# BaguaSys/bagua-core

Hardware: AMD Instinct MI355X
Metric: GiB/s fp32 gradient encode+decode (device-resident); 1/2/4/8-GPU compressed all-reduce GiB/s (higher is better)
Workload: dtype f32 -> u8

## Files before the change

bagua-core_amd/csrc/kernels/minmax_resident.hip:

```cpp
#include <hip/hip_runtime.h>
#include <stdio.h>
#include <stdlib.h>

#include <chrono>
#include <map>
#include <mutex>
#include <set>
#include <thread>
#include <utility>

#include "codec_common.hpp"
#include "launch_util.hpp"

namespace bagua {

constexpr int kResMaxGrid = 1024;
constexpr int kResSlots = 64;
constexpr int kResLanes = 8;

struct ResidentSlot {
    uint64_t ticket[kResLanes][16];
    uint64_t drained[kResLanes][16];
    uint64_t gave_up;
    uint64_t pad0[15];
    uint64_t gran[2 * kResMaxGrid];
};
static_assert(sizeof(ResidentSlot) % 64 == 0, "slot alignment");

struct ResidentArgs {
    const void* in;
    int64_t cs;
    int target;
    int nact;
    int bpc;
    int grid;
    uint8_t* out;
    int64_t chunk_offset;
    int64_t out_bytes;
    int num_chunks;
    ResidentSlot* slot;
    uint64_t timeout_ticks;
    uint64_t* trace;
};

__device__ __forceinline__ void trace_stamp(const ResidentArgs& a, int g, int k) {
    if (a.trace != nullptr && threadIdx.x == 0) a.trace[8 * g + k] = wall_clock64();
}

__device__ __forceinline__ uint32_t tag_of_ticket(uint64_t ticket, int grid, int lane) {
    const uint64_t per_launch = (uint64_t)((grid - lane + kResLanes - 1) / kResLanes);
    return (uint32_t)((ticket / per_launch) % 0xffffffffull) + 1u;
}

template <typename T, int BLOCK>
struct SliceGeom {
    using S = typename T::storage;
    int c;
    int cl;
    int b;
    const S* src;
    uint8_t* seg;
    uint8_t* payload;
    int64_t j0;
    int64_t nvec;
    int64_t v0, v1;
    bool last;

    __device__ __forceinline__ SliceGeom(const ResidentArgs& a, int g) {
        constexpr int N = Vec<T>::N;
        cl = g / a.bpc;
        b = g - cl * a.bpc;
        c = a.target < 0 ? cl : a.target;
        src = static_cast<const S*>(a.in) + (int64_t)c * a.cs;
        seg = a.out + (int64_t)c * a.chunk_offset;
        payload = seg + 32;
        const int al = common_alignment<T>((uintptr_t)src, (uintptr_t)payload);
        j0 = al < a.cs ? al : a.cs;
        nvec = (a.cs - j0) / N;
        const int64_t per = ((nvec + a.bpc - 1) / a.bpc + BLOCK - 1) / BLOCK * BLOCK;
        v0 = (int64_t)b * per;
        v0 = v0 < nvec ? v0 : nvec;
        v1 = v0 + per < nvec ? v0 + per : nvec;
        last = (b == a.bpc - 1);
    }
};

template <typename T>
__device__ __forceinline__ void fold_vec(const uint4& r, uint32_t& lo, uint32_t& hi) {
    float f[Vec<T>::N];
    unpack16<T>(r, f);
#pragma unroll
    for (int i = 0; i < Vec<T>::N; ++i) {
        const int32_t k = f2key(f[i]);
        lo = min(lo, min_space_key(k));
        hi = min(hi, max_space_key(k));
    }
}

template <typename T, int BLOCK>
__device__ __forceinline__ void fold_scalars(const ResidentArgs& a, const SliceGeom<T, BLOCK>& s, uint32_t& lo,
                                             uint32_t& hi) {
    constexpr int N = Vec<T>::N;
    const int t = (int)threadIdx.x;
    for (int64_t j = t; j < s.j0; j += BLOCK) {
        const int32_t k = f2key(T::to_f(s.src[j]));
        lo = min(lo, min_space_key(k));
        hi = min(hi, max_space_key(k));
    }
    for (int64_t j = s.j0 + s.nvec * N + t; j < a.cs; j += BLOCK) {
        const int32_t k = f2key(T::to_f(s.src[j]));
        lo = min(lo, min_space_key(k));
        hi = min(hi, max_space_key(k));
    }
}

template <int SB, int BLOCK, bool NT = false>
__device__ __forceinline__ void load_tile(const uint4* __restrict__ v, int64_t base, int t, uint4 (&r)[SB]) {
#pragma unroll
    for (int j = 0; j < SB; ++j) r[j] = NT ? nt_load16(&v[base + j * BLOCK + t]) : v[base + j * BLOCK + t];
}

template <typename T>
__device__ __forceinline__ void quant_store(const uint4& r, const QParams& q, uint8_t* dst) {
    float f[Vec<T>::N];
    unpack16<T>(r, f);
    quant_store_vec<T>(f, q, dst);
}

template <typename T, int BLOCK>
__device__ void write_extras(const ResidentArgs& a, const SliceGeom<T, BLOCK>& s, float mn, float mx,
                             const QParams& q) {
    using S = typename T::storage;
    constexpr int N = Vec<T>::N;
    const int t = (int)threadIdx.x;
    if (s.b == 0 && t < 32) {
        const uint32_t bmn = sizeof(S) == 4 ? __float_as_uint(mn) : (uint32_t)T::from_f(mn);
        const uint32_t bmx = sizeof(S) == 4 ? __float_as_uint(mx) : (uint32_t)T::from_f(mx);
        uint32_t hb = 0;
        if (t < (int)sizeof(S)) hb = (bmn >> (8 * t)) & 0xff;
        else if (t < 2 * (int)sizeof(S)) hb = (bmx >> (8 * (t - (int)sizeof(S)))) & 0xff;
        s.seg[t] = (uint8_t)hb;
    }
    if (!s.last) return;
    for (int64_t j = 32 + a.cs + t; j < a.chunk_offset; j += BLOCK) s.seg[j] = 0;
    if (a.target < 0 && s.c == a.num_chunks - 1)
        for (int64_t j = (int64_t)a.num_chunks * a.chunk_offset + t; j < a.out_bytes; j += BLOCK) a.out[j] = 0;
    for (int64_t j = t; j < s.j0; j += BLOCK) s.payload[j] = (uint8_t)quant(T::to_f(s.src[j]), q);
    for (int64_t j = s.j0 + s.nvec * N + t; j < a.cs; j += BLOCK)
        s.payload[j] = (uint8_t)quant(T::to_f(s.src[j]), q);
}

__device__ __forceinline__ bool sweep_chunk(const ResidentArgs& a, int cl, uint32_t tag, uint64_t deadline,
                                            uint32_t& lo, uint32_t& hi, bool bounded) {
    const int lane = lane_id();
    const uint64_t* g = a.slot->gran + 2 * (int64_t)cl * a.bpc;
    const int n = 2 * a.bpc;
    for (;;) {
        bool ok = true;
        uint32_t l = 0xffffffffu, h = 0xffffffffu;
        for (int i = lane; i < n; i += kWave) {
            const uint64_t x = __hip_atomic_load(g + i, __ATOMIC_RELAXED, __HIP_MEMORY_SCOPE_AGENT);
            ok &= (uint32_t)(x >> 32) == tag;
            if (i & 1) h = min(h, (uint32_t)x);
            else l = min(l, (uint32_t)x);
        }
        if (__all(ok)) {
            lo = wave_umin(l);
            hi = wave_umin(h);
            return true;
        }
        if (bounded && (uint64_t)wall_clock64() > deadline) return false;
        __builtin_amdgcn_s_sleep(2);
    }
}

template <typename T, int BLOCK, bool LEAN = false>
__device__ void fold_missing_slices(const ResidentArgs& a, int cl, uint32_t tag, uint32_t& lo, uint32_t& hi) {
    const int t = (int)threadIdx.x;
    for (int b = 0; b < a.bpc; ++b) {
        const int gg = cl * a.bpc + b;
        const uint64_t* gr = a.slot->gran + 2 * (int64_t)gg;
        const uint64_t x0 = __hip_atomic_load(gr, __ATOMIC_RELAXED, __HIP_MEMORY_SCOPE_AGENT);
        const uint64_t x1 = __hip_atomic_load(gr + 1, __ATOMIC_RELAXED, __HIP_MEMORY_SCOPE_AGENT);
        if ((uint32_t)(x0 >> 32) == tag && (uint32_t)(x1 >> 32) == tag) {
            lo = min(lo, (uint32_t)x0);
            hi = min(hi, (uint32_t)x1);
            continue;
        }
        const SliceGeom<T, BLOCK> sg(a, gg);
        const uint4* __restrict__ v = reinterpret_cast<const uint4*>(sg.src + sg.j0);
        if constexpr (LEAN) {
#pragma unroll 1
            for (int64_t i = sg.v0 + t; i < sg.v1; i += BLOCK) fold_vec<T>(v[i], lo, hi);
        } else {
            for (int64_t i = sg.v0 + t; i < sg.v1; i += BLOCK) fold_vec<T>(v[i], lo, hi);
        }
        if (sg.last) fold_scalars<T, BLOCK>(a, sg, lo, hi);
    }
}


template <int BLOCK>
__device__ __forceinline__ uint32_t draw_tag(const ResidentArgs& a, int lane_c, int t, uint32_t* scratch) {
    constexpr int W = BLOCK / kWave;
    if (t == 0) {
        const uint64_t ticket = __hip_atomic_fetch_add(&a.slot->ticket[lane_c][0], (uint64_t)1, __ATOMIC_RELAXED,
                                                       __HIP_MEMORY_SCOPE_AGENT);
        scratch[2 * W] = tag_of_ticket(ticket, a.grid, lane_c);
    }
    __syncthreads();
    return scratch[2 * W];
}

__device__ __forceinline__ void let_go_of_slot(const ResidentArgs& a, int lane_c, int t) {
    if (t == 0)
        __hip_atomic_fetch_add(&a.slot->drained[lane_c][0], (uint64_t)1, __ATOMIC_RELAXED,
                               __HIP_MEMORY_SCOPE_AGENT);
}

__device__ __forceinline__ void finish(const ResidentArgs& a, int g, int lane_c, int t) {
    if (a.trace != nullptr) {
        __syncthreads();
        trace_stamp(a, g, 3);
    }
    let_go_of_slot(a, lane_c, t);
}

template <int K, int ROW0, int BLOCK, bool NT, int M>
__device__ __forceinline__ void load_rows(const uint4* v, int64_t base, int64_t vl, int t,
                                          uint4 (&r)[M]) {
    static_assert(K <= M, "more rows than registers");
#pragma unroll
    for (int k = 0; k < K; ++k) {
        const int64_t i = base + (int64_t)(ROW0 + k) * BLOCK + t;
        r[k] = NT ? nt_load16(&v[i < vl ? i : vl]) : v[i < vl ? i : vl];
    }
}

template <typename T, int K, bool FENCE4, int M>
__device__ __forceinline__ void fold_rows(const uint4 (&r)[M], uint32_t& lo, uint32_t& hi) {
#pragma unroll
    for (int k = 0; k < K; ++k) {
        fold_vec<T>(r[k], lo, hi);
        if (FENCE4 && k % 4 == 3) __builtin_amdgcn_sched_barrier(0);
    }
}

template <typename T, int BLOCK, int H, int SB, int ROW0, bool NT>
__device__ __forceinline__ void fold_and_park(const uint4* v, int64_t v0, int64_t vl, int t,
                                              uint4 (&cur)[SB], uint4* park, uint32_t& lo, uint32_t& hi) {
    uint4 nxt[SB];
#pragma unroll
    for (int kb = 0; kb < H; kb += SB) {
#pragma unroll
        for (int j = 0; j < SB; ++j) {
            if (kb + SB + j < H) {
                const int64_t i = v0 + (int64_t)(ROW0 + kb + SB + j) * BLOCK + t;
                nxt[j] = NT ? nt_load16(&v[i < vl ? i : vl]) : v[i < vl ? i : vl];
            }
        }
#pragma unroll
        for (int j = 0; j < SB; ++j) {
            if (kb + j < H) {
                fold_vec<T>(cur[j], lo, hi);
                park[(kb + j) * BLOCK + t] = cur[j];
            }
        }
#pragma unroll
        for (int j = 0; j < SB; ++j) cur[j] = nxt[j];
    }
}

template <typename T, int BLOCK, int SB>
__device__ __forceinline__ void fold_stream_ascending(const uint4* v, int64_t stream0, int64_t nfull, int64_t last, int t,
                                                      uint4 (&ra)[SB], uint4 (&rb)[SB], uint32_t& lo,
                                                      uint32_t& hi) {
    constexpr int64_t tile = (int64_t)SB * BLOCK;
    for (int64_t i = 0; i < nfull; i += 2) {
        load_tile<SB, BLOCK>(v, stream0 + (i + 1 < nfull ? i + 1 : last) * tile, t, rb);
        fold_rows<T, SB, false>(ra, lo, hi);
        load_tile<SB, BLOCK>(v, stream0 + (i + 2 < nfull ? i + 2 : last) * tile, t, ra);
        if (i + 1 < nfull) fold_rows<T, SB, false>(rb, lo, hi);
    }
}

template <int BLOCK>
__device__ __forceinline__ void workgroup_umin(uint32_t& lo, uint32_t& hi, int t, int w, uint32_t* scratch) {
    constexpr int W = BLOCK / kWave;
    lo = wave_umin(lo);
    hi = wave_umin(hi);
    if (lane_id() == 0) { scratch[w] = lo; scratch[W + w] = hi; }
    __syncthreads();
    if (t == 0) {
#pragma unroll
        for (int i = 1; i < W; ++i) { lo = min(lo, scratch[i]); hi = min(hi, scratch[W + i]); }
    }
}

template <int BLOCK>
__device__ __forceinline__ void publish_partials(const ResidentArgs& a, int g, uint32_t tag, uint32_t lo, uint32_t hi,
                                                 int t, int w, uint32_t* scratch) {
    workgroup_umin<BLOCK>(lo, hi, t, w, scratch);
    if (t == 0) {
        uint64_t* mine = a.slot->gran + 2 * (int64_t)g;
        __hip_atomic_store(mine, ((uint64_t)tag << 32) | lo, __ATOMIC_RELAXED, __HIP_MEMORY_SCOPE_AGENT);
        __hip_atomic_store(mine + 1, ((uint64_t)tag << 32) | hi, __ATOMIC_RELAXED, __HIP_MEMORY_SCOPE_AGENT);
    }
}

struct MinMax {
    float mn, mx;
};

template <typename T, int BLOCK, bool LEAN>
__device__ __forceinline__ MinMax exchange_minmax(const ResidentArgs& a, int cl, uint32_t tag, int t, int w,
                                                  uint32_t* scratch) {
    constexpr int W = BLOCK / kWave;
    if (w == 0) {
        const uint64_t deadline = wall_clock64() + a.timeout_ticks;
        uint32_t l = 0, h = 0;
        const bool ok = sweep_chunk(a, cl, tag, deadline, l, h, true);
        if (lane_id() == 0) {
            scratch[2 * W + 1] = ok ? 1u : 0u;
            scratch[2 * W + 2] = l;
            scratch[2 * W + 3] = h;
        }
    }
    __syncthreads();
    if (scratch[2 * W + 1] == 0u) {
        if (t == 0) __hip_atomic_fetch_add(&a.slot->gave_up, (uint64_t)1, __ATOMIC_RELAXED, __HIP_MEMORY_SCOPE_AGENT);
        uint32_t l = 0xffffffffu, h = 0xffffffffu;
        fold_missing_slices<T, BLOCK, LEAN>(a, cl, tag, l, h);
        workgroup_umin<BLOCK>(l, h, t, w, scratch);
        if (t == 0) {
            scratch[2 * W + 2] = l;
            scratch[2 * W + 3] = h;
        }
        __syncthreads();
    }
    return MinMax{from_min_space(scratch[2 * W + 2]), from_max_space(scratch[2 * W + 3])};
}

template <int ON_CHIP>
__device__ __forceinline__ int on_chip_count(int64_t v0, int64_t v1) {
    return (int)(v1 - v0 < (int64_t)ON_CHIP ? (v1 > v0 ? v1 - v0 : 0) : (int64_t)ON_CHIP);
}

template <typename T, int BLOCK, int K, int ROW0, bool FENCE4, int M>
__device__ __forceinline__ void quant_rows(const uint4 (&r)[M], const QParams& q, uint8_t* vd) {
    constexpr int N = Vec<T>::N;
#pragma unroll
    for (int k = 0; k < K; ++k) {
        quant_store<T>(r[k], q, vd + (int64_t)(ROW0 + k) * BLOCK * N);
        if (FENCE4 && k % 4 == 3) __builtin_amdgcn_sched_barrier(0);
    }
}

template <typename T, int BLOCK, int K, int ROW0, int M>
__device__ __forceinline__ void quant_rows_guarded(const uint4 (&r)[M], int nloc, int t, const QParams& q,
                                                   uint8_t* vd) {
    constexpr int N = Vec<T>::N;
#pragma unroll
    for (int k = 0; k < K; ++k)
        if ((ROW0 + k) * BLOCK + t < nloc) quant_store<T>(r[k], q, vd + (int64_t)(ROW0 + k) * BLOCK * N);
}

template <typename T, int BLOCK, int H, int SB, int ROW0>
__device__ __forceinline__ void quant_parked(const uint4* park, int t, const QParams& q, uint8_t* vd) {
    constexpr int N = Vec<T>::N;
#pragma unroll
    for (int kb = 0; kb < H; kb += SB) {
        uint4 r[SB];
#pragma unroll
        for (int j = 0; j < SB; ++j)
            if (kb + j < H) r[j] = park[(kb + j) * BLOCK + t];
#pragma unroll
        for (int j = 0; j < SB; ++j)
            if (kb + j < H) quant_store<T>(r[j], q, vd + (int64_t)(ROW0 + kb + j) * BLOCK * N);
    }
}

template <typename T, int BLOCK, int H, int ROW0>
__device__ __forceinline__ void quant_parked_guarded(const uint4* park, int nloc, int t, const QParams& q,
                                                     uint8_t* vd) {
    constexpr int N = Vec<T>::N;
#pragma unroll
    for (int k = 0; k < H; ++k)
        if ((ROW0 + k) * BLOCK + t < nloc)
            quant_store<T>(park[k * BLOCK + t], q, vd + (int64_t)(ROW0 + k) * BLOCK * N);
}

template <typename T, int BLOCK, int SB>
__device__ __forceinline__ void quant_top_tile(const uint4 (&r)[SB], int64_t top, int64_t v1, int t,
                                               const QParams& q, uint8_t* vdst) {
    constexpr int N = Vec<T>::N;
#pragma unroll
    for (int j = 0; j < SB; ++j) {
        const int64_t i = top + j * BLOCK + t;
        if (i < v1) quant_store<T>(r[j], q, vdst + i * N);
    }
}

template <typename T, int BLOCK, int SB, bool NT>
__device__ __forceinline__ void quant_stream_descending(const uint4* v, int64_t stream0, int64_t nfull, int t,
                                                        const QParams& q, uint8_t* vdst, uint4 (&qa)[SB],
                                                        uint4 (&qb)[SB]) {
    constexpr int N = Vec<T>::N;
    constexpr int64_t tile = (int64_t)SB * BLOCK;
    for (int64_t i = nfull - 1; i >= 0; i -= 2) {
        load_tile<SB, BLOCK, NT>(v, stream0 + (i >= 1 ? i - 1 : 0) * tile, t, qb);
        const int64_t ba = stream0 + i * tile;
#pragma unroll
        for (int j = 0; j < SB; ++j) quant_store<T>(qa[j], q, vdst + (ba + j * BLOCK + t) * N);
        load_tile<SB, BLOCK, NT>(v, stream0 + (i >= 2 ? i - 2 : 0) * tile, t, qa);
        if (i >= 1) {
            const int64_t bb = ba - tile;
#pragma unroll
            for (int j = 0; j < SB; ++j) quant_store<T>(qb[j], q, vdst + (bb + j * BLOCK + t) * N);
        }
    }
}

template <typename T, int BLOCK, int SB, bool NT>
__device__ __forceinline__ void quant_stream_ascending(const uint4* v, int64_t stream0, int64_t nfull, int t,
                                                       const QParams& q, uint8_t* vdst, uint4 (&qa)[SB],
                                                       uint4 (&qb)[SB]) {
    constexpr int N = Vec<T>::N;
    constexpr int64_t tile = (int64_t)SB * BLOCK;
    for (int64_t i = 0; i < nfull; i += 2) {
        load_tile<SB, BLOCK, NT>(v, stream0 + (i + 1 < nfull ? i + 1 : nfull - 1) * tile, t, qb);
        const int64_t ba = stream0 + i * tile;
#pragma unroll
        for (int j = 0; j < SB; ++j) quant_store<T>(qa[j], q, vdst + (ba + j * BLOCK + t) * N);
        load_tile<SB, BLOCK, NT>(v, stream0 + (i + 2 < nfull ? i + 2 : nfull - 1) * tile, t, qa);
        if (i + 1 < nfull) {
            const int64_t bb = ba + tile;
#pragma unroll
            for (int j = 0; j < SB; ++j) quant_store<T>(qb[j], q, vdst + (bb + j * BLOCK + t) * N);
        }
    }
}

template <typename T, int BLOCK, int R, int H, int SB, int NTM>
__global__ __launch_bounds__(BLOCK, 1) void minmax_resident_encode_kernel(ResidentArgs a) {
    constexpr int N = Vec<T>::N;
    constexpr bool NT = (NTM & 1) != 0;
    constexpr bool NT1 = (NTM & 2) != 0;
    extern __shared__ __attribute__((aligned(16))) uint4 smem[];
    uint4* park = smem;
    uint32_t* scratch = reinterpret_cast<uint32_t*>(smem + H * BLOCK);
    const int t = (int)threadIdx.x;
    const int g = (int)blockIdx.x;
    const int lane_c = g % kResLanes;

    const uint32_t tag = draw_tag<BLOCK>(a, lane_c, t, scratch);
    trace_stamp(a, g, 0);
    if (g >= a.nact * a.bpc) {
        let_go_of_slot(a, lane_c, t);
        return;
    }

    const SliceGeom<T, BLOCK> s(a, g);
    const uint4* __restrict__ v = reinterpret_cast<const uint4*>(s.src + s.j0);
    const int64_t v0 = s.v0, v1 = s.v1;
    const int64_t stream0 = v0 + (int64_t)(R + H) * BLOCK;

    uint32_t lo = min_space(T::init_max());
    uint32_t hi = max_space(-T::init_max());
    uint4 held[R > 0 ? R : 1];
    if (v1 > v0) {
        const int64_t vl = v1 - 1;
        load_rows<R, 0, BLOCK, NT1>(v, v0, vl, t, held);
        uint4 cur[SB];
        load_rows<(H < SB ? H : SB), R, BLOCK, NT1>(v, v0, vl, t, cur);
        fold_rows<T, R, false>(held, lo, hi);
        fold_and_park<T, BLOCK, H, SB, R, NT1>(v, v0, vl, t, cur, park, lo, hi);
        const int64_t tile = (int64_t)SB * BLOCK;
        const int64_t nfull = v1 > stream0 ? (v1 - stream0) / tile : 0;
        if (nfull > 0) {
            uint4 ra[SB], rb[SB];
            load_tile<SB, BLOCK>(v, stream0, t, ra);
            fold_stream_ascending<T, BLOCK, SB>(v, stream0, nfull, nfull - 1, t, ra, rb, lo, hi);
        }
        for (int j = 0; j < SB; ++j) {
            const int64_t i = stream0 + nfull * tile + j * BLOCK + t;
            if (i < v1) fold_vec<T>(v[i], lo, hi);
        }
    }
    if (s.last) fold_scalars<T, BLOCK>(a, s, lo, hi);
    const int w = t / kWave;
    publish_partials<BLOCK>(a, g, tag, lo, hi, t, w, scratch);

    const int64_t tile2 = (int64_t)SB * BLOCK;
    const int64_t nfull2 = v1 > stream0 ? (v1 - stream0) / tile2 : 0;
    uint4 pre[SB], pre2[SB];
    if (nfull2 > 0) load_tile<SB, BLOCK, NT>(v, stream0 + (nfull2 - 1) * tile2, t, pre);
    if (nfull2 > 1) load_tile<SB, BLOCK, NT>(v, stream0 + (nfull2 - 2) * tile2, t, pre2);

    trace_stamp(a, g, 1);
    const MinMax m = exchange_minmax<T, BLOCK, false>(a, s.cl, tag, t, w, scratch);
    const QParams q = make_qparams(m.mn, m.mx);
    trace_stamp(a, g, 2);

    write_extras<T, BLOCK>(a, s, m.mn, m.mx, q);
    uint8_t* vdst = s.payload + s.j0;
    if (v1 > stream0) {
        const int64_t tile = (int64_t)SB * BLOCK;
        const int64_t nfull = (v1 - stream0) / tile;
        for (int j = 0; j < SB; ++j) {
            const int64_t i = stream0 + nfull * tile + j * BLOCK + t;
            if (i < v1) quant_store<T>(v[i], q, vdst + i * N);
        }
        if (nfull > 0) {
            uint4 ra[SB], rb[SB];
#pragma unroll
            for (int j = 0; j < SB; ++j) { ra[j] = pre[j]; rb[j] = pre2[j]; }
            for (int64_t i = nfull - 1; i >= 0; i -= 2) {
                if (i != nfull - 1 || nfull < 2) load_tile<SB, BLOCK, NT>(v, stream0 + (i >= 1 ? i - 1 : 0) * tile, t, rb);
                const int64_t ba = stream0 + i * tile;
#pragma unroll
                for (int j = 0; j < SB; ++j) quant_store<T>(ra[j], q, vdst + (ba + j * BLOCK + t) * N);
                load_tile<SB, BLOCK, NT>(v, stream0 + (i >= 2 ? i - 2 : 0) * tile, t, ra);
                if (i >= 1) {
                    const int64_t bb = ba - tile;
#pragma unroll
                    for (int j = 0; j < SB; ++j) quant_store<T>(rb[j], q, vdst + (bb + j * BLOCK + t) * N);
                }
            }
        }
    }
    trace_stamp(a, g, 4);
    if (v0 + (int64_t)(R + H) * BLOCK <= v1) {
        uint8_t* vd = vdst + (v0 + t) * N;
        quant_parked<T, BLOCK, H, SB, R>(park, t, q, vd);
        trace_stamp(a, g, 5);
        quant_rows<T, BLOCK, R, 0, false>(held, q, vd);
    } else {
#pragma unroll
        for (int k = 0; k < H; ++k) {
            const int64_t i = v0 + (int64_t)(R + k) * BLOCK + t;
            if (i < v1) quant_store<T>(park[k * BLOCK + t], q, vdst + i * N);
        }
        trace_stamp(a, g, 5);
#pragma unroll
        for (int k = 0; k < R; ++k) {
            const int64_t i = v0 + (int64_t)k * BLOCK + t;
            if (i < v1) quant_store<T>(held[k], q, vdst + i * N);
        }
    }
    finish(a, g, lane_c, t);
}

template <typename T, int BLOCK, int R, int H, int SB, int NTM, bool EARLY, bool ASC>
__global__ __launch_bounds__(BLOCK, 1) void minmax_resident_encode_kernel_stack(ResidentArgs a) {
    constexpr int N = Vec<T>::N;
    constexpr bool NT = (NTM & 1) != 0;
    constexpr bool NT1 = (NTM & 2) != 0;
    static_assert(R > 0 && H > 0, "the stack order keeps rows in VGPRs and in LDS");
    extern __shared__ __attribute__((aligned(16))) uint4 smem[];
    uint4* park = smem;
    uint32_t* scratch = reinterpret_cast<uint32_t*>(smem + H * BLOCK);
    const int t = (int)threadIdx.x;
    const int g = (int)blockIdx.x;
    const int lane_c = g % kResLanes;
    const bool idle = g >= a.nact * a.bpc;

    const SliceGeom<T, BLOCK> s(a, idle ? 0 : g);
    const uint4* __restrict__ v = reinterpret_cast<const uint4*>(s.src + s.j0);
    const int64_t v0 = s.v0, v1 = s.v1;
    const int64_t vl = v1 - 1;
    const int64_t stream0 = v0 + (int64_t)(R + H) * BLOCK;
    const int64_t tile = (int64_t)SB * BLOCK;
    const int64_t nfull = v1 > stream0 ? (v1 - stream0) / tile : 0;
    const int64_t top = stream0 + nfull * tile;

    uint4 ra[SB];
    if (EARLY && !idle && nfull > 0) load_tile<SB, BLOCK>(v, stream0, t, ra);
    const uint32_t tag = draw_tag<BLOCK>(a, lane_c, t, scratch);
    trace_stamp(a, g, 0);
    if (idle) {
        let_go_of_slot(a, lane_c, t);
        return;
    }

    uint32_t lo = min_space(T::init_max());
    uint32_t hi = max_space(-T::init_max());
    uint4 held[R];
    if (v1 > v0) {
        uint4 rb[SB];
        if (nfull > 0) {
            if (!EARLY) load_tile<SB, BLOCK>(v, stream0, t, ra);
            fold_stream_ascending<T, BLOCK, SB>(v, stream0, nfull, nfull - 1, t, ra, rb, lo, hi);
        }
        uint4 cur[SB];
        if (v1 > top) load_rows<SB, 0, BLOCK, false>(v, top, vl, t, rb);
        load_rows<(H < SB ? H : SB), R, BLOCK, NT1>(v, v0, vl, t, cur);
        if (v1 > top) fold_rows<T, SB, false>(rb, lo, hi);
        fold_and_park<T, BLOCK, H, SB, R, NT1>(v, v0, vl, t, cur, park, lo, hi);
        __builtin_amdgcn_sched_barrier(0);
        load_rows<R, 0, BLOCK, NT1>(v, v0, vl, t, held);
        __builtin_amdgcn_sched_barrier(0);
        fold_rows<T, R, true>(held, lo, hi);
    }
    if (s.last) fold_scalars<T, BLOCK>(a, s, lo, hi);
    const int w = t / kWave;
    publish_partials<BLOCK>(a, g, tag, lo, hi, t, w, scratch);
    trace_stamp(a, g, 1);

    constexpr int W = BLOCK / kWave;
    if (w == 0) {
        const uint64_t deadline = wall_clock64() + a.timeout_ticks;
        uint32_t l = 0, h = 0;
        const bool ok = sweep_chunk(a, s.cl, tag, deadline, l, h, true);
        if (lane_id() == 0) {
            scratch[2 * W + 1] = ok ? 1u : 0u;
            scratch[2 * W + 2] = l;
            scratch[2 * W + 3] = h;
        }
    }
    __syncthreads();
    if (scratch[2 * W + 1] == 0u) {
        if (t == 0) __hip_atomic_fetch_add(&a.slot->gave_up, (uint64_t)1, __ATOMIC_RELAXED, __HIP_MEMORY_SCOPE_AGENT);
        uint32_t l = 0xffffffffu, h = 0xffffffffu;
        fold_missing_slices<T, BLOCK, true>(a, s.cl, tag, l, h);
        workgroup_umin<BLOCK>(l, h, t, w, scratch);
        if (t == 0) {
            scratch[2 * W + 2] = l;
            scratch[2 * W + 3] = h;
        }
        __syncthreads();
    }
    const MinMax m{from_min_space(scratch[2 * W + 2]), from_max_space(scratch[2 * W + 3])};
    const QParams q = make_qparams(m.mn, m.mx);
    trace_stamp(a, g, 2);

    write_extras<T, BLOCK>(a, s, m.mn, m.mx, q);
    uint8_t* vdst = s.payload + s.j0;
    const bool whole = stream0 <= v1;
    uint8_t* vd = vdst + (v0 + t) * N;
    const int nloc = on_chip_count<(R + H) * BLOCK>(v0, v1);
    if (whole) quant_rows<T, BLOCK, R, 0, true>(held, q, vd);
    else quant_rows_guarded<T, BLOCK, R, 0>(held, nloc, t, q, vd);
    __builtin_amdgcn_sched_barrier(0);
    trace_stamp(a, g, 6);
    uint4 qa[SB], qb[SB];
    if (v1 > top) load_rows<SB, 0, BLOCK, NT>(v, top, vl, t, qb);
    if (nfull > 0) load_tile<SB, BLOCK, NT>(v, stream0 + (ASC ? 0 : nfull - 1) * tile, t, qa);
    if (whole) quant_parked<T, BLOCK, H, SB, R>(park, t, q, vd);
    else quant_parked_guarded<T, BLOCK, H, R>(park, nloc, t, q, vd);
    trace_stamp(a, g, 7);
    if (v1 > top) quant_top_tile<T, BLOCK, SB>(qb, top, v1, t, q, vdst);
    if (ASC && nfull > 0) quant_stream_ascending<T, BLOCK, SB, NT>(v, stream0, nfull, t, q, vdst, qa, qb);
    else if (nfull > 0) quant_stream_descending<T, BLOCK, SB, NT>(v, stream0, nfull, t, q, vdst, qa, qb);
    finish(a, g, lane_c, t);
}

template <typename T, int BLOCK, int RE, int H, int RL, int SB, int NTM>
__global__ __launch_bounds__(BLOCK, 1) void minmax_resident_encode_kernel_window(ResidentArgs a) {
    constexpr int N = Vec<T>::N;
    constexpr bool NT = (NTM & 1) != 0;
    constexpr bool NT1 = (NTM & 2) != 0;
    static_assert(RE > 0 && H > 0 && RL > 0, "the window order keeps rows in VGPRs (early and late) and in LDS");
    extern __shared__ __attribute__((aligned(16))) uint4 smem[];
    uint4* park = smem;
    uint32_t* scratch = reinterpret_cast<uint32_t*>(smem + H * BLOCK);
    const int t = (int)threadIdx.x;
    const int g = (int)blockIdx.x;
    const int lane_c = g % kResLanes;

    const uint32_t tag = draw_tag<BLOCK>(a, lane_c, t, scratch);
    trace_stamp(a, g, 0);
    if (g >= a.nact * a.bpc) {
        let_go_of_slot(a, lane_c, t);
        return;
    }

    const SliceGeom<T, BLOCK> s(a, g);
    const uint4* __restrict__ v = reinterpret_cast<const uint4*>(s.src + s.j0);
    const int64_t v0 = s.v0, v1 = s.v1;
    const int64_t vl = v1 - 1;
    const int64_t stream0 = v0 + (int64_t)(RE + H + RL) * BLOCK;
    const int64_t tile = (int64_t)SB * BLOCK;
    const int64_t nfull = v1 > stream0 ? (v1 - stream0) / tile : 0;
    const int64_t top = stream0 + nfull * tile;

    uint32_t lo = min_space(T::init_max());
    uint32_t hi = max_space(-T::init_max());
    uint4 held[RE], late[RL];
    if (v1 > v0) {
        load_rows<RE, 0, BLOCK, NT1>(v, v0, vl, t, held);
        uint4 cur[SB];
        load_rows<(H < SB ? H : SB), RE, BLOCK, NT1>(v, v0, vl, t, cur);
        fold_rows<T, RE, true>(held, lo, hi);
        fold_and_park<T, BLOCK, H, SB, RE, NT1>(v, v0, vl, t, cur, park, lo, hi);
        uint4 ra[SB], rb[SB];
        if (nfull > 0) {
            load_tile<SB, BLOCK>(v, stream0, t, ra);
            fold_stream_ascending<T, BLOCK, SB>(v, stream0, nfull, nfull - 1, t, ra, rb, lo, hi);
        }
        if (v1 > top) {
            load_rows<SB, 0, BLOCK, false>(v, top, vl, t, rb);
            fold_rows<T, SB, false>(rb, lo, hi);
        }
        __builtin_amdgcn_sched_barrier(0);
        load_rows<RL, RE + H, BLOCK, NT1>(v, v0, vl, t, late);
        __builtin_amdgcn_sched_barrier(0);
        fold_rows<T, RL, true>(late, lo, hi);
    }
    if (s.last) fold_scalars<T, BLOCK>(a, s, lo, hi);
    const int w = t / kWave;
    publish_partials<BLOCK>(a, g, tag, lo, hi, t, w, scratch);
    trace_stamp(a, g, 1);

    const MinMax m = exchange_minmax<T, BLOCK, true>(a, s.cl, tag, t, w, scratch);
    const QParams q = make_qparams(m.mn, m.mx);
    trace_stamp(a, g, 2);

    write_extras<T, BLOCK>(a, s, m.mn, m.mx, q);
    uint8_t* vdst = s.payload + s.j0;
    const bool whole = stream0 <= v1;
    uint8_t* vd = vdst + (v0 + t) * N;
    const int nloc = on_chip_count<(RE + H + RL) * BLOCK>(v0, v1);
    if (whole) quant_rows<T, BLOCK, RL, RE + H, true>(late, q, vd);
    else quant_rows_guarded<T, BLOCK, RL, RE + H>(late, nloc, t, q, vd);
    __builtin_amdgcn_sched_barrier(0);
    trace_stamp(a, g, 6);
    {
        uint4 qa[SB], qb[SB];
        if (v1 > top) load_rows<SB, 0, BLOCK, NT>(v, top, vl, t, qb);
        if (nfull > 0) load_tile<SB, BLOCK, NT>(v, stream0 + (nfull - 1) * tile, t, qa);
        if (v1 > top) quant_top_tile<T, BLOCK, SB>(qb, top, v1, t, q, vdst);
        if (nfull > 0) quant_stream_descending<T, BLOCK, SB, NT>(v, stream0, nfull, t, q, vdst, qa, qb);
    }
    __builtin_amdgcn_sched_barrier(0);
    trace_stamp(a, g, 4);
    if (whole) {
        quant_parked<T, BLOCK, H, SB, RE>(park, t, q, vd);
        trace_stamp(a, g, 5);
        quant_rows<T, BLOCK, RE, 0, true>(held, q, vd);
    } else {
        quant_parked_guarded<T, BLOCK, H, RE>(park, nloc, t, q, vd);
        trace_stamp(a, g, 5);
        quant_rows_guarded<T, BLOCK, RE, 0>(held, nloc, t, q, vd);
    }
    finish(a, g, lane_c, t);
}

struct StreamKey {
    hipStream_t s = nullptr;
    std::thread::id tid{};
    bool operator<(const StreamKey& o) const { return s != o.s ? s < o.s : tid < o.tid; }
    bool operator==(const StreamKey& o) const { return s == o.s && tid == o.tid; }
};
static StreamKey stream_key(hipStream_t s) {
    StreamKey k;
    k.s = s;
    if (s == hipStreamPerThread) k.tid = std::this_thread::get_id();
    return k;
}

struct SlotState {
    bool used = false;
    bool captured = false;
    StreamKey owner;
    uint64_t last_use = 0;
    uint64_t launched = 0;
};

struct ResidentDevice {
    bool init = false, ok = false;
    int grid = 0;
    int clock_khz = 0;
    ResidentSlot* slots = nullptr;
    uint64_t* probe_host = nullptr;
    SlotState state[kResSlots];
    std::map<StreamKey, int> stream_slot;
    uint64_t clock = 0;
    bool warned_full = false;
};
static std::mutex g_res_mu;
static std::set<hipStream_t>& resident_off_streams() {
    static auto* s = new std::set<hipStream_t>();
    return *s;
}
static uint64_t* g_res_trace = nullptr;
static ResidentDevice g_res_dev[64];

struct ResidentCfg {
    int block, r, h, sb;
    int ntm;
    int stack;
    int rl;
};
static constexpr ResidentCfg kResCfg[] = {
    {256, 32, 39, 8, 0},
    {256, 48, 39, 8, 0},
    {512, 24, 19, 8, 0},
    {256, 0, 0, 8, 0},
    {256, 32, 0, 8, 0},
    {256, 16, 39, 16, 0},
    {256, 64, 39, 8, 0},
    {256, 80, 39, 8, 0},
    {256, 72, 39, 8, 0},
    {512, 28, 19, 8, 0},
    {256, 80, 39, 8, 1},
    {512, 28, 19, 8, 1},
    {512, 28, 19, 8, 3},
    {512, 28, 19, 8, 2},
    {512, 40, 19, 8, 3, 1},
    {512, 44, 19, 8, 3, 1},
    {512, 48, 19, 8, 3, 1},
    {512, 52, 19, 4, 3, 1},
    {512, 48, 19, 4, 3, 1},
    {512, 52, 19, 4, 3, 3},
    {512, 28, 19, 8, 3, 1},
    {512, 48, 19, 8, 3, 3},
    {512, 44, 19, 8, 3, 3},
    {512, 52, 19, 4, 3, 5},
    {512, 52, 19, 4, 3, 7},
    {512, 52, 19, 4, 1, 1},
    {512, 52, 19, 4, 1, 5},
    {512, 48, 19, 4, 3, 5},
    {512, 44, 19, 4, 3, 5},
    {512, 44, 19, 4, 3, 1},
    {512, 44, 19, 4, 3, 0},
    {512, 44, 19, 4, 3, 0, 8},
    {512, 40, 19, 4, 3, 0, 12},
};
constexpr int kResNumCfg = (int)(sizeof(kResCfg) / sizeof(kResCfg[0]));
static_assert(kResCfg[29].rl == 0 && kResCfg[31].rl == 8 && kResCfg[32].rl == 12, "row numbers are named by BAGUA_RESIDENT_CFG and the tests");
template <typename T>
constexpr int resident_default_cfg();
template <>
constexpr int resident_default_cfg<F32>() {
    return 32;
}
template <>
constexpr int resident_default_cfg<BF16>() {
    return 31;
}
template <>
constexpr int resident_default_cfg<F16>() {
    return 29;
}

static size_t resident_lds_bytes(const ResidentCfg& c) {
    return (size_t)c.h * c.block * 16 + 16 * ((2 * (c.block / kWave) + 4 + 3) / 4);
}

using ResidentKernel = void (*)(ResidentArgs);

template <typename T, int CFG>
static ResidentKernel resident_kernel_ptr() {
    constexpr ResidentCfg c = kResCfg[CFG];
    if constexpr (c.rl != 0)
        return &minmax_resident_encode_kernel_window<T, c.block, c.r, c.h, c.rl, c.sb, c.ntm>;
    else if constexpr (c.stack != 0)
        return &minmax_resident_encode_kernel_stack<T, c.block, c.r, c.h, c.sb, c.ntm, (c.stack & 2) != 0,
                                                    (c.stack & 4) != 0>;
    else
        return &minmax_resident_encode_kernel<T, c.block, c.r, c.h, c.sb, c.ntm>;
}

template <typename T, size_t... I>
static ResidentKernel resident_kernel_at(int cfg, std::index_sequence<I...>) {
    static const ResidentKernel table[] = {resident_kernel_ptr<T, (int)I>()...};
    return table[cfg];
}

template <typename T>
static ResidentKernel resident_kernel_for(int cfg) {
    if (cfg < 0 || cfg >= kResNumCfg) return nullptr;
    return resident_kernel_at<T>(cfg, std::make_index_sequence<kResNumCfg>{});
}

static bool device_ready(int dev) {
    if (dev < 0 || dev >= 64) return false;
    ResidentDevice& d = g_res_dev[dev];
    if (!d.init) {
        d.init = true;
        int cus = 0, khz = 0;
        if (hipDeviceGetAttribute(&cus, hipDeviceAttributeMultiprocessorCount, dev) != hipSuccess) return false;
        if (hipDeviceGetAttribute(&khz, hipDeviceAttributeWallClockRate, dev) != hipSuccess) return false;
        if (cus < 1 || cus > kResMaxGrid || khz < 1) return false;
        void* p = nullptr;
        const size_t bytes = sizeof(ResidentSlot) * kResSlots;
        if (hipMalloc(&p, bytes) != hipSuccess) return false;
        if (hipMemset(p, 0, bytes) != hipSuccess || hipDeviceSynchronize() != hipSuccess) {
            (void)hipFree(p);
            return false;
        }
        void* h = nullptr;
        if (hipHostMalloc(&h, sizeof(ResidentSlot::drained), hipHostMallocDefault) != hipSuccess) {
            (void)hipFree(p);
            return false;
        }
        d.probe_host = static_cast<uint64_t*>(h);
        d.slots = static_cast<ResidentSlot*>(p);
        d.grid = cus;
        d.clock_khz = khz;
        d.ok = true;
    }
    return d.ok;
}

static int wait_slot_drained(int dev, int idx, hipStream_t via) {
    ResidentDevice& d = g_res_dev[dev];
    const uint64_t want = d.state[idx].launched;
    for (;;) {
        if (hipMemcpyAsync(d.probe_host, &d.slots[idx].drained[0][0], sizeof(ResidentSlot::drained),
                           hipMemcpyDeviceToHost, via) != hipSuccess ||
            hipStreamSynchronize(via) != hipSuccess) {
            g_last_hip_error = (int)hipGetLastError();
            return BAGUA_ERR_HIP;
        }
        uint64_t got = 0;
        for (int c = 0; c < kResLanes; ++c) got += d.probe_host[16 * c];
        if (got >= want) return BAGUA_OK;
        std::this_thread::sleep_for(std::chrono::microseconds(20));
    }
}

static int acquire_slot_locked(int dev, hipStream_t s) {
    ResidentDevice& d = g_res_dev[dev];
    const StreamKey key = stream_key(s);
    int idx = -1;
    auto it = d.stream_slot.find(key);
    if (it != d.stream_slot.end()) {
        idx = it->second;
    } else {
        for (int i = 0; i < kResSlots && idx < 0; ++i)
            if (!d.state[i].used && !d.state[i].captured) idx = i;
        if (idx < 0) {
            for (int i = 0; i < kResSlots; ++i)
                if (!d.state[i].captured && (idx < 0 || d.state[i].last_use < d.state[idx].last_use)) idx = i;
            if (idx < 0) return -1;
            SlotState& old = d.state[idx];
            if (wait_slot_drained(dev, idx, s) != BAGUA_OK) return -1;
            d.stream_slot.erase(old.owner);
            if (!d.warned_full) {
                d.warned_full = true;
                fprintf(stderr,
                        "[bagua-core] one-launch encode: %d streams in use on device %d; reclaiming the least "
                        "recently used slot (release streams with bagua_minmax_u8_release_stream)\n",
                        kResSlots, dev);
            }
        }
        SlotState& st = d.state[idx];
        st.used = true;
        st.owner = key;
        d.stream_slot.emplace(key, idx);
    }
    d.state[idx].last_use = ++d.clock;
    return idx;
}

struct ResidentPlan {
    bool ok = false;
    ResidentKernel kern = nullptr;
    int block = 0;
    int dev = 0;
    size_t lds = 0;
    ResidentArgs a{};
};

template <typename T>
static ResidentPlan resident_plan(const void* input, int64_t in_num_elem, int64_t cs, int p, uint8_t* out,
                                  int64_t out_bytes, int target, hipStream_t s) {
    using S = typename T::storage;
    ResidentPlan pl;
    const int cfg = tune_int("BAGUA_RESIDENT_CFG", resident_default_cfg<T>());
    if (tune_int("BAGUA_RESIDENT", 1) == 0 || cfg < 0 || cfg >= kResNumCfg || p <= 0) return pl;
    {
        std::lock_guard<std::mutex> lk(g_res_mu);
        if (resident_off_streams().count(s)) return pl;
    }
    const int nact = target < 0 ? p : 1;
    const int64_t chunk_offset = out_bytes / p;
    if (in_num_elem < (target < 0 ? (int64_t)p * cs : ((int64_t)target + 1) * cs)) return pl;
    if (cs * nact < tune_int("BAGUA_RESIDENT_MIN_ELEMS", 12 << 20)) return pl;
    for (int i = 0; i < nact; ++i) {
        const int c = target < 0 ? i : target;
        const uintptr_t src = (uintptr_t)(static_cast<const S*>(input) + (int64_t)c * cs);
        const uintptr_t pay = (uintptr_t)(out + (int64_t)c * chunk_offset + 32);
        if (src % sizeof(S) != 0 || common_alignment<T>(src, pay) < 0) return pl;
    }
    int dev = 0;
    if (hipGetDevice(&dev) != hipSuccess || dev < 0 || dev >= 64) return pl;
    int grid = 0, khz = 0;
    {
        std::lock_guard<std::mutex> lk(g_res_mu);
        if (!device_ready(dev)) return pl;
        grid = g_res_dev[dev].grid;
        khz = g_res_dev[dev].clock_khz;
    }
    if (nact > grid) return pl;
    const ResidentCfg& c = kResCfg[cfg];
    const ResidentKernel kern = resident_kernel_for<T>(cfg);
    const void* kfn = reinterpret_cast<const void*>(kern);
    const size_t lds = resident_lds_bytes(c);
    {
        static int admitted[64][kResNumCfg];
        std::lock_guard<std::mutex> lk(g_res_mu);
        int& st = admitted[dev][cfg];
        if (st == 0) {
            int per_cu = 0;
            st = (hipFuncSetAttribute(kfn, hipFuncAttributeMaxDynamicSharedMemorySize, (int)lds) == hipSuccess &&
                  hipOccupancyMaxActiveBlocksPerMultiprocessor(&per_cu, kfn, c.block, lds) == hipSuccess &&
                  per_cu >= 1)
                     ? 1
                     : -1;
            (void)hipGetLastError();
        }
        if (st < 0) return pl;
    }
    ResidentArgs& a = pl.a;
    a.in = input;
    a.cs = cs;
    a.target = target;
    a.nact = nact;
    a.bpc = grid / nact;
    a.grid = grid;
    a.out = out;
    a.chunk_offset = chunk_offset;
    a.out_bytes = out_bytes;
    a.num_chunks = p;
    a.slot = nullptr;
    const int64_t active_bytes = cs * nact * (int64_t)sizeof(S);
    const int64_t us = tune_int("BAGUA_RESIDENT_TIMEOUT_US", (int)(200 + active_bytes / 500000));
    a.timeout_ticks = (uint64_t)(us < 0 ? 0 : us) * (uint64_t)khz / 1000u;
    a.trace = g_res_trace;
    pl.kern = kern;
    pl.block = c.block;
    pl.lds = lds;
    pl.dev = dev;
    pl.ok = true;
    return pl;
}

template <typename T>
int resident_compress_impl(const void* input, int64_t in_num_elem, int64_t cs, int p, uint8_t* out,
                           int64_t out_bytes, int target, hipStream_t s) {
    ResidentPlan pl = resident_plan<T>(input, in_num_elem, cs, p, out, out_bytes, target, s);
    if (!pl.ok) return BAGUA_ERR_UNSUPPORTED;
    std::lock_guard<std::mutex> lk(g_res_mu);
    ResidentDevice& d = g_res_dev[pl.dev];
    const int idx = acquire_slot_locked(pl.dev, s);
    if (idx < 0) return BAGUA_ERR_UNSUPPORTED;
    hipStreamCaptureStatus cap = hipStreamCaptureStatusNone;
    if (hipStreamIsCapturing(s, &cap) != hipSuccess) (void)hipGetLastError();
    if (cap != hipStreamCaptureStatusNone) d.state[idx].captured = true;
    pl.a.slot = d.slots + idx;
    const ResidentArgs& a = pl.a;
    launch(pl.kern, dim3(a.grid), dim3(pl.block), (uint32_t)pl.lds, s, a);
    const int rc = check_launch();
    if (rc == BAGUA_OK) d.state[idx].launched += (uint64_t)a.grid;
    return rc;
}

int release_stream_slot(hipStream_t s) {
    std::lock_guard<std::mutex> lk(g_res_mu);
    const StreamKey key = stream_key(s);
    int rc = BAGUA_OK;
    for (int dev = 0; dev < 64; ++dev) {
        ResidentDevice& d = g_res_dev[dev];
        if (!d.ok) continue;
        auto it = d.stream_slot.find(key);
        if (it == d.stream_slot.end()) continue;
        SlotState& st = d.state[it->second];
        if (st.captured) {
            d.stream_slot.erase(it);
            continue;
        }
        if (wait_slot_drained(dev, it->second, s) != BAGUA_OK) {
            rc = BAGUA_ERR_HIP;
            continue;
        }
        st.used = false;
        st.last_use = 0;
        d.stream_slot.erase(it);
    }
    return rc;
}

int resident_give_ups(hipStream_t s, uint64_t* count) {
    std::lock_guard<std::mutex> lk(g_res_mu);
    *count = 0;
    int dev = 0;
    if (hipGetDevice(&dev) != hipSuccess || dev < 0 || dev >= 64 || !g_res_dev[dev].ok) return BAGUA_OK;
    ResidentDevice& d = g_res_dev[dev];
    auto it = d.stream_slot.find(stream_key(s));
    if (it == d.stream_slot.end()) return BAGUA_OK;
    if (hipMemcpyAsync(d.probe_host, &d.slots[it->second].gave_up, sizeof(uint64_t), hipMemcpyDeviceToHost, s) !=
            hipSuccess ||
        hipStreamSynchronize(s) != hipSuccess) {
        g_last_hip_error = (int)hipGetLastError();
        return BAGUA_ERR_HIP;
    }
    *count = *d.probe_host;
    return BAGUA_OK;
}

int resident_slots_in_use(int dev) {
    std::lock_guard<std::mutex> lk(g_res_mu);
    if (dev < 0 || dev >= 64 || !g_res_dev[dev].ok) return 0;
    return (int)g_res_dev[dev].stream_slot.size();
}

template <typename T>
int resident_eligible(const void* input, int64_t in_num_elem, int64_t cs, int p, uint8_t* out, int64_t out_bytes,
                      int target, hipStream_t s) {
    return resident_plan<T>(input, in_num_elem, cs, p, out, out_bytes, target, s).ok ? 1 : 0;
}

template int resident_compress_impl<F32>(const void*, int64_t, int64_t, int, uint8_t*, int64_t, int, hipStream_t);
template int resident_compress_impl<F16>(const void*, int64_t, int64_t, int, uint8_t*, int64_t, int, hipStream_t);
template int resident_compress_impl<BF16>(const void*, int64_t, int64_t, int, uint8_t*, int64_t, int, hipStream_t);

}

extern "C" int bagua_minmax_u8_release_stream(bagua_stream_t stream) {
    {
        std::lock_guard<std::mutex> lk(bagua::g_res_mu);
        bagua::resident_off_streams().erase(static_cast<hipStream_t>(stream));
    }
    return bagua::release_stream_slot(static_cast<hipStream_t>(stream));
}

extern "C" int bagua_minmax_u8_set_stream_resident(bagua_stream_t stream, int allowed) {
    std::lock_guard<std::mutex> lk(bagua::g_res_mu);
    if (allowed) bagua::resident_off_streams().erase(static_cast<hipStream_t>(stream));
    else bagua::resident_off_streams().insert(static_cast<hipStream_t>(stream));
    return BAGUA_OK;
}

extern "C" int bagua_minmax_u8_resident_slots_in_use(int device_id) { return bagua::resident_slots_in_use(device_id); }

extern "C" int bagua_minmax_u8_resident_give_ups(bagua_stream_t stream, uint64_t* count) {
    if (!count) return BAGUA_ERR_INVALID_ARG;
    return bagua::resident_give_ups(static_cast<hipStream_t>(stream), count);
}

extern "C" int bagua_minmax_u8_resident_trace(void* device_buffer) {
    std::lock_guard<std::mutex> lk(bagua::g_res_mu);
    bagua::g_res_trace = static_cast<uint64_t*>(device_buffer);
    return BAGUA_OK;
}

extern "C" int bagua_minmax_u8_resident_path(int dtype, const void* input, int input_num_element, int chunk_size,
                                             int num_chunks, uint8_t* output, size_t output_bytes, int target_chunk,
// ... 69 lines not shown
```

Measured before the change: 1999.

## Defer ticket tag resolution off the critical path and split chunk sweep across waves

The entry-point __syncthreads after the ticket atomic is removed; the ticket is drawn asynchronously and its tag is parked in LDS, then read back after the later workgroup reduction barrier, so its latency overlaps with loads. The cross-block min/max sweep now runs on two waves with batched, per-element retry polling instead of one wave re-reading everything. Tag computation gets a 32-bit fast path to avoid a 64-bit divide. It adds LDS scratch words and more complex bookkeeping, and the entry trace stamp is deferred.

```diff
diff --git a/bagua-core_amd/csrc/kernels/minmax_resident.hip b/bagua-core_amd/csrc/kernels/minmax_resident.hip
--- a/bagua-core_amd/csrc/kernels/minmax_resident.hip
+++ b/bagua-core_amd/csrc/kernels/minmax_resident.hip
@@ -48,8 +48,12 @@
 }
 
 __device__ __forceinline__ uint32_t tag_of_ticket(uint64_t ticket, int grid, int lane) {
-    const uint64_t per_launch = (uint64_t)((grid - lane + kResLanes - 1) / kResLanes);
-    return (uint32_t)((ticket / per_launch) % 0xffffffffull) + 1u;
+    const uint32_t per_launch = (uint32_t)((grid - lane + kResLanes - 1) / kResLanes);
+    if ((ticket >> 32) == 0) {
+        const uint32_t k = (uint32_t)ticket / per_launch;
+        return (k == 0xffffffffu ? 0u : k) + 1u;
+    }
+    return (uint32_t)((ticket / (uint64_t)per_launch) % 0xffffffffull) + 1u;
 }
 
 template <typename T, int BLOCK>
@@ -150,28 +154,44 @@
         s.payload[j] = (uint8_t)quant(T::to_f(s.src[j]), q);
 }
 
-__device__ __forceinline__ bool sweep_chunk(const ResidentArgs& a, int cl, uint32_t tag, uint64_t deadline,
+constexpr int kSweepWaves = 2;
+constexpr int kSweepBatch = 4;
+__device__ __forceinline__ bool sweep_chunk(const ResidentArgs& a, int cl, uint32_t tag, int w, uint64_t deadline,
                                             uint32_t& lo, uint32_t& hi, bool bounded) {
     const int lane = lane_id();
     const uint64_t* g = a.slot->gran + 2 * (int64_t)cl * a.bpc;
     const int n = 2 * a.bpc;
-    for (;;) {
-        bool ok = true;
-        uint32_t l = 0xffffffffu, h = 0xffffffffu;
-        for (int i = lane; i < n; i += kWave) {
-            const uint64_t x = __hip_atomic_load(g + i, __ATOMIC_RELAXED, __HIP_MEMORY_SCOPE_AGENT);
-            ok &= (uint32_t)(x >> 32) == tag;
-            if (i & 1) h = min(h, (uint32_t)x);
-            else l = min(l, (uint32_t)x);
-        }
-        if (__all(ok)) {
-            lo = wave_umin(l);
-            hi = wave_umin(h);
-            return true;
-        }
-        if (bounded && (uint64_t)wall_clock64() > deadline) return false;
-        __builtin_amdgcn_s_sleep(2);
-    }
+    const int first = w * kWave + lane;
+    uint32_t key = 0xffffffffu;
+    for (int base = first; base - first < n; base += kSweepBatch * kSweepWaves * kWave) {
+        uint32_t missing = 0;
+#pragma unroll
+        for (int j = 0; j < kSweepBatch; ++j)
+            if (base + j * kSweepWaves * kWave < n) missing |= 1u << j;
+        for (;;) {
+            uint64_t x[kSweepBatch];
+#pragma unroll
+            for (int j = 0; j < kSweepBatch; ++j) {
+                x[j] = 0;
+                if ((missing >> j) & 1u)
+                    x[j] = __hip_atomic_load(g + (uint32_t)(base + j * kSweepWaves * kWave), __ATOMIC_RELAXED,
+                                             __HIP_MEMORY_SCOPE_AGENT);
+            }
+#pragma unroll
+            for (int j = 0; j < kSweepBatch; ++j) {
+                if ((uint32_t)(x[j] >> 32) == tag) {
+                    key = min(key, (uint32_t)x[j]);
+                    missing &= ~(1u << j);
+                }
+            }
+            if (__all(missing == 0)) break;
+            if (bounded && (uint64_t)wall_clock64() > deadline) return false;
+            __builtin_amdgcn_s_sleep(2);
+        }
+    }
+    lo = wave_umin((lane & 1) ? 0xffffffffu : key);
+    hi = wave_umin((lane & 1) ? key : 0xffffffffu);
+    return true;
 }
 
 template <typename T, int BLOCK, bool LEAN = false>
@@ -199,17 +219,45 @@
     }
 }
 
+constexpr int res_scratch_words(int block) { return 2 * (block / kWave) + 2 + 2 * kSweepWaves + 2; }
 
 template <int BLOCK>
-__device__ __forceinline__ uint32_t draw_tag(const ResidentArgs& a, int lane_c, int t, uint32_t* scratch) {
+__device__ __forceinline__ void trace_entry(const ResidentArgs& a, int t, uint32_t* scratch) {
+    constexpr int W = BLOCK / kWave;
+    if (a.trace != nullptr && t == 0) {
+        const uint64_t now = wall_clock64();
+        scratch[2 * W + 2 + 2 * kSweepWaves] = (uint32_t)now;
+        scratch[2 * W + 3 + 2 * kSweepWaves] = (uint32_t)(now >> 32);
+    }
+}
+
+template <int BLOCK>
+__device__ __forceinline__ void trace_entry_flush(const ResidentArgs& a, int g, int t,
+                                                  const uint32_t* scratch) {
+    constexpr int W = BLOCK / kWave;
+    if (a.trace != nullptr && t == 0)
+        a.trace[8 * g] = ((uint64_t)scratch[2 * W + 3 + 2 * kSweepWaves] << 32) | scratch[2 * W + 2 + 2 * kSweepWaves];
+}
+
+__device__ __forceinline__ uint64_t draw_ticket(const ResidentArgs& a, int lane_c, int t) {
+    uint64_t ticket = 0;
+    if (t == 0) {
+        int zero = 0;
+        asm volatile("" : "+v"(zero));
+        ticket = __hip_atomic_fetch_add(&a.slot->ticket[lane_c][zero], (uint64_t)1, __ATOMIC_RELAXED,
+                                        __HIP_MEMORY_SCOPE_AGENT);
+    }
+    return ticket;
+}
+
+template <int BLOCK>
+__device__ __forceinline__ void park_tag(const ResidentArgs& a, uint64_t ticket, int lane_c, int t,
+                                         uint32_t* scratch) {
     constexpr int W = BLOCK / kWave;
     if (t == 0) {
-        const uint64_t ticket = __hip_atomic_fetch_add(&a.slot->ticket[lane_c][0], (uint64_t)1, __ATOMIC_RELAXED,
-                                                       __HIP_MEMORY_SCOPE_AGENT);
         scratch[2 * W] = tag_of_ticket(ticket, a.grid, lane_c);
-    }
-    __syncthreads();
-    return scratch[2 * W];
+        scratch[2 * W + 1] = 1u;
+    }
 }
 
 __device__ __forceinline__ void let_go_of_slot(const ResidentArgs& a, int lane_c, int t) {
@@ -298,14 +346,17 @@
 }
 
 template <int BLOCK>
-__device__ __forceinline__ void publish_partials(const ResidentArgs& a, int g, uint32_t tag, uint32_t lo, uint32_t hi,
-                                                 int t, int w, uint32_t* scratch) {
+__device__ __forceinline__ uint32_t publish_partials(const ResidentArgs& a, int g, uint32_t lo, uint32_t hi,
+                                                     int t, int w, uint32_t* scratch) {
+    constexpr int W = BLOCK / kWave;
     workgroup_umin<BLOCK>(lo, hi, t, w, scratch);
+    const uint32_t tag = scratch[2 * W];
     if (t == 0) {
         uint64_t* mine = a.slot->gran + 2 * (int64_t)g;
         __hip_atomic_store(mine, ((uint64_t)tag << 32) | lo, __ATOMIC_RELAXED, __HIP_MEMORY_SCOPE_AGENT);
         __hip_atomic_store(mine + 1, ((uint64_t)tag << 32) | hi, __ATOMIC_RELAXED, __HIP_MEMORY_SCOPE_AGENT);
     }
+    return tag;
 }
 
 struct MinMax {
@@ -316,14 +367,14 @@
 __device__ __forceinline__ MinMax exchange_minmax(const ResidentArgs& a, int cl, uint32_t tag, int t, int w,
                                                   uint32_t* scratch) {
     constexpr int W = BLOCK / kWave;
-    if (w == 0) {
+    if (w < kSweepWaves) {
         const uint64_t deadline = wall_clock64() + a.timeout_ticks;
         uint32_t l = 0, h = 0;
-        const bool ok = sweep_chunk(a, cl, tag, deadline, l, h, true);
+        const bool ok = sweep_chunk(a, cl, tag, w, deadline, l, h, true);
         if (lane_id() == 0) {
-            scratch[2 * W + 1] = ok ? 1u : 0u;
-            scratch[2 * W + 2] = l;
-            scratch[2 * W + 3] = h;
+            if (!ok) scratch[2 * W + 1] = 0u;
+            scratch[2 * W + 2 + 2 * w] = l;
+            scratch[2 * W + 3 + 2 * w] = h;
         }
     }
     __syncthreads();
@@ -333,12 +384,21 @@
         fold_missing_slices<T, BLOCK, LEAN>(a, cl, tag, l, h);
         workgroup_umin<BLOCK>(l, h, t, w, scratch);
         if (t == 0) {
-            scratch[2 * W + 2] = l;
-            scratch[2 * W + 3] = h;
+#pragma unroll
+            for (int i = 0; i < kSweepWaves; ++i) {
+                scratch[2 * W + 2 + 2 * i] = l;
+                scratch[2 * W + 3 + 2 * i] = h;
+            }
         }
         __syncthreads();
     }
-    return MinMax{from_min_space(scratch[2 * W + 2]), from_max_space(scratch[2 * W + 3])};
+    uint32_t cmin = scratch[2 * W + 2], cmax = scratch[2 * W + 3];
+#pragma unroll
+    for (int i = 1; i < kSweepWaves; ++i) {
+        cmin = min(cmin, scratch[2 * W + 2 + 2 * i]);
+        cmax = min(cmax, scratch[2 * W + 3 + 2 * i]);
+    }
+    return MinMax{from_min_space(cmin), from_max_space(cmax)};
 }
 
 template <int ON_CHIP>
@@ -453,12 +513,14 @@
     const int g = (int)blockIdx.x;
     const int lane_c = g % kResLanes;
 
-    const uint32_t tag = draw_tag<BLOCK>(a, lane_c, t, scratch);
-    trace_stamp(a, g, 0);
+    trace_entry<BLOCK>(a, t, scratch);
+    const uint64_t ticket = draw_ticket(a, lane_c, t);
     if (g >= a.nact * a.bpc) {
+        trace_entry_flush<BLOCK>(a, g, t, scratch);
         let_go_of_slot(a, lane_c, t);
         return;
     }
+    park_tag<BLOCK>(a, ticket, lane_c, t, scratch);
 
     const SliceGeom<T, BLOCK> s(a, g);
     const uint4* __restrict__ v = reinterpret_cast<const uint4*>(s.src + s.j0);
@@ -489,7 +551,7 @@
     }
     if (s.last) fold_scalars<T, BLOCK>(a, s, lo, hi);
     const int w = t / kWave;
-    publish_partials<BLOCK>(a, g, tag, lo, hi, t, w, scratch);
+    const uint32_t tag = publish_partials<BLOCK>(a, g, lo, hi, t, w, scratch);
 
     const int64_t tile2 = (int64_t)SB * BLOCK;
     const int64_t nfull2 = v1 > stream0 ? (v1 - stream0) / tile2 : 0;
@@ -497,6 +559,7 @@
     if (nfull2 > 0) load_tile<SB, BLOCK, NT>(v, stream0 + (nfull2 - 1) * tile2, t, pre);
     if (nfull2 > 1) load_tile<SB, BLOCK, NT>(v, stream0 + (nfull2 - 2) * tile2, t, pre2);
 
+    trace_entry_flush<BLOCK>(a, g, t, scratch);
     trace_stamp(a, g, 1);
     const MinMax m = exchange_minmax<T, BLOCK, false>(a, s.cl, tag, t, w, scratch);
     const QParams q = make_qparams(m.mn, m.mx);
@@ -575,10 +638,11 @@
     const int64_t top = stream0 + nfull * tile;
 
     uint4 ra[SB];
+    trace_entry<BLOCK>(a, t, scratch);
     if (EARLY && !idle && nfull > 0) load_tile<SB, BLOCK>(v, stream0, t, ra);
-    const uint32_t tag = draw_tag<BLOCK>(a, lane_c, t, scratch);
-    trace_stamp(a, g, 0);
+    const uint64_t ticket = draw_ticket(a, lane_c, t);
     if (idle) {
+        trace_entry_flush<BLOCK>(a, g, t, scratch);
         let_go_of_slot(a, lane_c, t);
         return;
     }
@@ -588,10 +652,9 @@
     uint4 held[R];
     if (v1 > v0) {
         uint4 rb[SB];
-        if (nfull > 0) {
-            if (!EARLY) load_tile<SB, BLOCK>(v, stream0, t, ra);
-            fold_stream_ascending<T, BLOCK, SB>(v, stream0, nfull, nfull - 1, t, ra, rb, lo, hi);
-        }
+        if (!EARLY && nfull > 0) load_tile<SB, BLOCK>(v, stream0, t, ra);
+        park_tag<BLOCK>(a, ticket, lane_c, t, scratch);
+        if (nfull > 0) fold_stream_ascending<T, BLOCK, SB>(v, stream0, nfull, nfull - 1, t, ra, rb, lo, hi);
         uint4 cur[SB];
         if (v1 > top) load_rows<SB, 0, BLOCK, false>(v, top, vl, t, rb);
         load_rows<(H < SB ? H : SB), R, BLOCK, NT1>(v, v0, vl, t, cur);
@@ -601,21 +664,24 @@
         load_rows<R, 0, BLOCK, NT1>(v, v0, vl, t, held);
         __builtin_amdgcn_sched_barrier(0);
         fold_rows<T, R, true>(held, lo, hi);
+    } else {
+        park_tag<BLOCK>(a, ticket, lane_c, t, scratch);
     }
     if (s.last) fold_scalars<T, BLOCK>(a, s, lo, hi);
     const int w = t / kWave;
-    publish_partials<BLOCK>(a, g, tag, lo, hi, t, w, scratch);
+    const uint32_t tag = publish_partials<BLOCK>(a, g, lo, hi, t, w, scratch);
+    trace_entry_flush<BLOCK>(a, g, t, scratch);
     trace_stamp(a, g, 1);
 
     constexpr int W = BLOCK / kWave;
-    if (w == 0) {
+    if (w < kSweepWaves) {
         const uint64_t deadline = wall_clock64() + a.timeout_ticks;
         uint32_t l = 0, h = 0;
-        const bool ok = sweep_chunk(a, s.cl, tag, deadline, l, h, true);
+        const bool ok = sweep_chunk(a, s.cl, tag, w, deadline, l, h, true);
         if (lane_id() == 0) {
-            scratch[2 * W + 1] = ok ? 1u : 0u;
-            scratch[2 * W + 2] = l;
-            scratch[2 * W + 3] = h;
+            if (!ok) scratch[2 * W + 1] = 0u;
+            scratch[2 * W + 2 + 2 * w] = l;
+            scratch[2 * W + 3 + 2 * w] = h;
         }
     }
     __syncthreads();
@@ -625,12 +691,21 @@
         fold_missing_slices<T, BLOCK, true>(a, s.cl, tag, l, h);
         workgroup_umin<BLOCK>(l, h, t, w, scratch);
         if (t == 0) {
-            scratch[2 * W + 2] = l;
-            scratch[2 * W + 3] = h;
+#pragma unroll
+            for (int i = 0; i < kSweepWaves; ++i) {
+                scratch[2 * W + 2 + 2 * i] = l;
+                scratch[2 * W + 3 + 2 * i] = h;
+            }
         }
         __syncthreads();
     }
-    const MinMax m{from_min_space(scratch[2 * W + 2]), from_max_space(scratch[2 * W + 3])};
+    uint32_t cmin = scratch[2 * W + 2], cmax = scratch[2 * W + 3];
+#pragma unroll
+    for (int i = 1; i < kSweepWaves; ++i) {
+        cmin = min(cmin, scratch[2 * W + 2 + 2 * i]);
+        cmax = min(cmax, scratch[2 * W + 3 + 2 * i]);
+    }
+    const MinMax m{from_min_space(cmin), from_max_space(cmax)};
     const QParams q = make_qparams(m.mn, m.mx);
     trace_stamp(a, g, 2);
 
@@ -668,12 +743,14 @@
     const int g = (int)blockIdx.x;
     const int lane_c = g % kResLanes;
 
-    const uint32_t tag = draw_tag<BLOCK>(a, lane_c, t, scratch);
-    trace_stamp(a, g, 0);
+    trace_entry<BLOCK>(a, t, scratch);
+    const uint64_t ticket = draw_ticket(a, lane_c, t);
     if (g >= a.nact * a.bpc) {
+        trace_entry_flush<BLOCK>(a, g, t, scratch);
         let_go_of_slot(a, lane_c, t);
         return;
     }
+    park_tag<BLOCK>(a, ticket, lane_c, t, scratch);
 
     const SliceGeom<T, BLOCK> s(a, g);
     const uint4* __restrict__ v = reinterpret_cast<const uint4*>(s.src + s.j0);
@@ -709,7 +786,8 @@
     }
     if (s.last) fold_scalars<T, BLOCK>(a, s, lo, hi);
     const int w = t / kWave;
-    publish_partials<BLOCK>(a, g, tag, lo, hi, t, w, scratch);
+    const uint32_t tag = publish_partials<BLOCK>(a, g, lo, hi, t, w, scratch);
+    trace_entry_flush<BLOCK>(a, g, t, scratch);
     trace_stamp(a, g, 1);
 
     const MinMax m = exchange_minmax<T, BLOCK, true>(a, s.cl, tag, t, w, scratch);
@@ -845,7 +923,7 @@
 }
 
 static size_t resident_lds_bytes(const ResidentCfg& c) {
-    return (size_t)c.h * c.block * 16 + 16 * ((2 * (c.block / kWave) + 4 + 3) / 4);
+    return (size_t)c.h * c.block * 16 + 16 * ((size_t)(res_scratch_words(c.block) + 3) / 4);
 }
 
 using ResidentKernel = void (*)(ResidentArgs);
```

Measured after the change: 2024, median of 6. +1.3%, better.
